# adityamwagh/SuperSLAM

Hardware: AMD Instinct MI355X
Metric: stereo pairs/sec (SPx2+LG) at 1376x376 (higher is better)
Workload: dtype f16; 1 GPU; configs[1]: SuperPoint x2 + select + gather + 1x LightGlue on 1376x376 stereo pairs; a step = 8 x 64 = 512 pairs per GPU resident in HBM (8 library calls of 64 pairs, different images per call), max_keypoints 600, seeded synthetic weights; pairs_per_call=64, max_keypoints=600, matches_last_call=1412, parallelism=replicated weights, pairs sharded over 1 rank(s), no data-path collective

## Files before the change

superslam_amd/csrc/api.hip:

```cpp
#include <algorithm>
#include <atomic>
#include <cmath>
#include <cstdarg>
#include <cstdlib>
#include <cstring>
#include <fstream>
#include <map>
#include <memory>
#include <mutex>
#include <string>
#include <vector>

#include "../../include/sship.h"
#include "../../include/superslam_hip/place_recognizer.hpp"
#include "kernels.h"

namespace sship {

static thread_local std::string g_err;
static void (*g_log_cb)(int, const char*) = nullptr;
static int g_profiling = 0;

void set_error(const std::string& msg) {
  g_err = msg;
// ... 572 lines not shown
}

static int conv_mode() {
  static const int v = [] {
    const char* e = dev_env("SUPERSLAM_HIP_CONV");
    return (SSHIP_DEV_SWITCHES && e && std::string(e) == "strip") ? 2 : 1;
  }();
  return v;
}
static hipError_t conv3(const ConvW& w, const _Float16* in, _Float16* out, int B, int H, int W, bool pool, hipStream_t s) {
#if SSHIP_DEV_SWITCHES
  static const bool wino = [] { const char* e = dev_env("SUPERSLAM_HIP_CONV64"); return e && std::string(e) == "wino"; }();
  if (wino && w.w_wino && sp_conv3x3_wino_fits(H, W, w.cin, w.cout)) return sp_conv3x3_wino(w.w_wino, w.bias, in, out, B, H, W, pool, s);
  return conv_mode() == 1 ? sp_conv3x3_pp(w, in, out, B, H, W, pool, s) : sp_conv3x3_strip(w, in, out, B, H, W, pool, s);
#else
  return sp_conv3x3_pp(w, in, out, B, H, W, pool, s);
#endif
}
static bool conv2_fused(int B, int H2, int W2) {
#if SSHIP_DEV_SWITCHES
  static const std::string mode = [] { const char* e = dev_env("SUPERSLAM_HIP_CONV2"); return std::string(e ? e : ""); }();
  static const bool other = [] { const char* e = dev_env("SUPERSLAM_HIP_CONV64"); return e != nullptr; }();
  if (mode == "split" || other || conv_mode() != 1) return false;
#endif
  return sp_conv2ab_fused_fits(B, H2, W2, true);
}
static hipError_t conv3a_layer(const ConvW& w, const _Float16* in, _Float16* out, int B, int H, int W, hipStream_t s) {
#if SSHIP_DEV_SWITCHES
  static const bool roll = [] { const char* e = dev_env("SUPERSLAM_HIP_CONV3A"); return e && std::string(e) == "roll"; }();
  if (roll && conv_mode() == 1 && w.cin == 64 && w.cout == 128 && w.ct == 64 && sp_conv3a_roll_fits(B, H, W)) return sp_conv3a_roll(w, in, out, B, H, W, s);
#endif
  return conv3(w, in, out, B, H, W, false, s);
}
static hipError_t conv1ab(sship_sp* sp, const uint8_t* img, _Float16* out, int B, int H, int W, hipStream_t s);
static bool desc_dense_mode() {
  static const bool v = [] { const char* e = dev_env("SUPERSLAM_HIP_DESC"); return e && std::string(e) == "dense"; }();
  return v;
}
static hipError_t desc_head(sship_sp* sp, int img0, int Hc, int Wc, const int* cell_h, const int* cell_w, const int* n_dev, int B,
                            _Float16* out, size_t out_img_stride, hipStream_t s) {
  const int mk = sp->cfg.max_keypoints;
  if (desc_dense_mode()) {
    launch_desc_head_gather(sp->cDb32, sp->aDa.as<_Float16>() + (size_t)img0 * Hc * Wc * 256, Hc, Wc, cell_h, cell_w, n_dev, mk, B, out,
                            out_img_stride, s);
    return hipGetLastError();
  }
  return launch_desc_head_sparse(sp->cDa, sp->cDb32, sp->a4b.as<_Float16>() + (size_t)img0 * Hc * Wc * 128, Hc, Wc, cell_h, cell_w, n_dev,
                                 mk, B, out, out_img_stride, s);
}

static int sp_network(sship_sp* sp, const uint8_t* imgs, int B, int H, int W, hipStream_t s, bool dense_desc) {
  int H2, W2, H4, W4, Hc, Wc;
  sp_shapes(H, W, H2, W2, H4, W4, Hc, Wc);
  SSHIP_HIP_CHECK(conv1ab(sp, imgs, sp->a1b.as<_Float16>(), B, H, W, s));
  g_timer.mark_fine("sp_gpu_infer:encoder/conv1a+conv1b+pool", s);
  if (conv2_fused(B, H2, W2)) {
    SSHIP_HIP_CHECK(sp_conv2ab_fused(sp->c2a, sp->c2b, sp->a1b.as<_Float16>(), sp->a2b.as<_Float16>(), B, H2, W2, s));
    g_timer.mark_fine("sp_gpu_infer:encoder/conv2a+conv2b+pool", s);
  } else {
    SSHIP_HIP_CHECK(conv3(sp->c2a, sp->a1b.as<_Float16>(), sp->a2a.as<_Float16>(), B, H2, W2, false, s));
    g_timer.mark_fine("sp_gpu_infer:encoder/conv2a", s);
    SSHIP_HIP_CHECK(conv3(sp->c2b, sp->a2a.as<_Float16>(), sp->a2b.as<_Float16>(), B, H2, W2, true, s));
    g_timer.mark_fine("sp_gpu_infer:encoder/conv2b+pool", s);
  }
  SSHIP_HIP_CHECK(conv3a_layer(sp->c3a, sp->a2b.as<_Float16>(), sp->a3a.as<_Float16>(), B, H4, W4, s));
  g_timer.mark_fine("sp_gpu_infer:encoder/conv3a", s);
  SSHIP_HIP_CHECK(conv3(sp->c3b, sp->a3a.as<_Float16>(), sp->a3b.as<_Float16>(), B, H4, W4, true, s));
  g_timer.mark_fine("sp_gpu_infer:encoder/conv3b+pool", s);
  SSHIP_HIP_CHECK(conv3(sp->c4a, sp->a3b.as<_Float16>(), sp->a4a.as<_Float16>(), B, Hc, Wc, false, s));
  g_timer.mark_fine("sp_gpu_infer:encoder/conv4a", s);
  SSHIP_HIP_CHECK(conv3(sp->c4b, sp->a4a.as<_Float16>(), sp->a4b.as<_Float16>(), B, Hc, Wc, false, s));
  g_timer.mark(g_profiling >= 2 ? "sp_gpu_infer:encoder/conv4b" : "sp_gpu_infer:encoder", s);
  SSHIP_HIP_CHECK(conv3(sp->cPa, sp->a4b.as<_Float16>(), sp->aPa.as<_Float16>(), B, Hc, Wc, false, s));
  g_timer.mark_fine("sp_gpu_infer:heads/convPa", s);
  SSHIP_HIP_CHECK(sp_conv1x1_f32(sp->cPb, sp->aPa.as<_Float16>(), sp->logits.as<float>(), kLogitStride, B, Hc, Wc, s));
  if (dense_desc || desc_dense_mode()) SSHIP_HIP_CHECK(conv3(sp->cDa, sp->a4b.as<_Float16>(), sp->aDa.as<_Float16>(), B, Hc, Wc, false, s));
  if (dense_desc) SSHIP_HIP_CHECK(sp_conv1x1_f16(sp->cDb, sp->aDa.as<_Float16>(), sp->draw.as<_Float16>(), B, Hc, Wc, s));
  g_timer.mark(g_profiling >= 2 ? "sp_gpu_infer:heads/convPb" : "sp_gpu_infer:heads", s);
  return SSHIP_OK;
}

static int sp_select(sship_sp* sp, int B, int H, int W, float* scores_out, float* kp_out, int* n_out, hipStream_t s) {
  int H2, W2, H4, W4, Hc, Wc;
  sp_shapes(H, W, H2, W2, H4, W4, Hc, Wc);
  if (sp->cand_zero_ptr != sp->cand_count.p || sp->cand_zero_n < B || sp->cand_zero_stream != s)
    SSHIP_HIP_CHECK(hipMemsetAsync(sp->cand_count.p, 0, (size_t)B * 4, s));
  sp->cand_zero_ptr = sp->cand_count.p; sp->cand_zero_n = 0; sp->cand_zero_stream = s;
  NmsArgs a{};
  a.logits = sp->logits.as<float>(); a.ls = kLogitStride; a.B = B; a.H = Hc * 8; a.W = Wc * 8;
  a.radius = sp->cfg.nms_radius; a.thr_f = sp->thr_f; a.border = sp->cfg.remove_borders;
  a.cand = sp->cand.as<unsigned long long>(); a.cand_count = sp->cand_count.as<int>(); a.cap = sp->cap;
  a.scores_out = scores_out;
  launch_nms_tile(0, a, s);
  g_timer.mark_fine("sp_extract_stereo:select/nms_tile", s);
  TopkArgs t{};
  t.cand = a.cand; t.cand_count = a.cand_count; t.cap = sp->cap; t.max_kp = sp->cfg.max_keypoints;
  t.score_w = Wc * 8;
  t.scale_x = static_cast<float>(W) / (Wc * 8);
  t.scale_y = static_cast<float>(H) / (Hc * 8);
  t.desc_h = Hc; t.desc_w = Wc; t.kp_xys = kp_out; t.cell_h = sp->cell_h.as<int>(); t.cell_w = sp->cell_w.as<int>();
  t.n_out = n_out; t.n_cand_out = nullptr; t.reset_count = a.cand_count;
  launch_topk(t, B, s);
  SSHIP_HIP_CHECK(hipGetLastError());
  sp->cand_zero_n = B;
  g_timer.mark(g_profiling >= 2 ? "sp_extract_stereo:select/topk" : "sp_extract_stereo:select", s);
  return SSHIP_OK;
}

static hipError_t conv1ab(sship_sp* sp, const uint8_t* img, _Float16* out, int B, int H, int W, hipStream_t s) {
#if SSHIP_DEV_SWITCHES
  if (conv_mode() == 2) return sp_conv1ab_fused(sp->c1b, sp->w1a_frag, sp->b1a, img, out, B, H, W, s);
// ... 73 lines not shown
          const _Float16 hi = (_Float16)b->data[co];
          f[4] = hi;
          f[5] = (_Float16)(b->data[co] - (float)hi);
        }
      }
    SSHIP_HIP_CHECK(hipMalloc(reinterpret_cast<void**>(&sp->w1a_fragb), fr.size() * sizeof(_Float16)));
    SSHIP_HIP_CHECK(hipMemcpy(sp->w1a_fragb, fr.data(), fr.size() * sizeof(_Float16), hipMemcpyHostToDevice));
  }
  SSHIP_HIP_CHECK(hipStreamCreateWithFlags(&sp->stream, hipStreamDefault));
  if (int rc = sship_pool_create(sp->cfg.pool_slots, sp->cfg.max_keypoints, SSHIP_DESC_DIM, &sp->pool)) return rc;
  *out = sp.release();
  return SSHIP_OK;
}
extern "C" void sship_sp_destroy(sship_sp* sp) {
  bind_thread();
  if (!sp) return;
  (void)hipDeviceSynchronize();
  for (ConvW* c : {&sp->c1b, &sp->c2a, &sp->c2b, &sp->c3a, &sp->c3b, &sp->c4a, &sp->c4b, &sp->cPa, &sp->cPb, &sp->cDa, &sp->cDb, &sp->cDb32})
    free_conv(*c);
  if (sp->w1a) (void)hipFree(sp->w1a);
  if (sp->b1a) (void)hipFree(sp->b1a);
  if (sp->w1a_frag) (void)hipFree(sp->w1a_frag);
  if (sp->w1a_fragb) (void)hipFree(sp->w1a_fragb);
  ring_free(sp);
  if (sp->pool) sship_pool_destroy(sp->pool);
  sp->pool = nullptr;
  if (sp->stream) (void)hipStreamDestroy(sp->stream);
  delete sp;
}
extern "C" int sship_sp_debug_activation(sship_sp* sp, int layer, void* out_host, unsigned long long bytes) {
  bind_thread();
  if (!sp || !out_host) return fail(SSHIP_ERR_INVALID, "sp_debug_activation: null argument");
  DevBuf* bufs[8] = {nullptr, &sp->a1b, &sp->a2a, &sp->a2b, &sp->a3a, &sp->a3b, &sp->a4a, &sp->a4b};
  if (layer < 1 || layer > 7 || !bufs[layer]->p || bytes > bufs[layer]->bytes) return fail(SSHIP_ERR_INVALID, "sp_debug_activation: bad layer / size");
  SSHIP_HIP_CHECK(hipDeviceSynchronize());
  SSHIP_HIP_CHECK(hipMemcpy(out_host, bufs[layer]->p, bytes, hipMemcpyDeviceToHost));
  return SSHIP_OK;
}
extern "C" sship_pool* sship_sp_pool(sship_sp* sp) {
  bind_thread(); return sp ? sp->pool : nullptr; }
extern "C" int sship_sp_max_keypoints(const sship_sp* sp) { return sp ? sp->cfg.max_keypoints : 0; }

extern "C" int sship_sp_extract_batch_device(sship_sp* sp, const uint8_t* imgs, int batch, int h, int w, void* desc_out,
                                             float* kp_out, int* n_out, void* stream) {
  bind_thread();
  if (!sp || !imgs || !desc_out || !kp_out || !n_out || batch <= 0) return fail(SSHIP_ERR_INVALID, "sp_extract_batch_device: bad arguments");
  hipStream_t s = static_cast<hipStream_t>(stream);
  if (int rc = sp_ensure(sp, batch, h, w)) return rc;
  if (g_profiling && imgs != sp->img.as<uint8_t>())
    SSHIP_HIP_CHECK(hipMemcpyAsync(sp->img.p, imgs, (size_t)batch * h * w, hipMemcpyDeviceToDevice, s));
  sp->img_valid = g_profiling != 0 || imgs == sp->img.as<uint8_t>();
  g_timer.begin(s);
  if (int rc = sp_network(sp, imgs, batch, h, w, s, false)) return rc;
  if (int rc = sp_select(sp, batch, h, w, nullptr, kp_out, n_out, s)) return rc;
  int H2, W2, H4, W4, Hc, Wc;
  sp_shapes(h, w, H2, W2, H4, W4, Hc, Wc);
  SSHIP_HIP_CHECK(desc_head(sp, 0, Hc, Wc, sp->cell_h.as<int>(), sp->cell_w.as<int>(), n_out, batch, static_cast<_Float16*>(desc_out),
                            (size_t)sp->cfg.max_keypoints * 256, s));
  g_timer.mark("sp_extract_stereo:gather", s);
  return SSHIP_OK;
}

extern "C" int sship_sp_dense(sship_sp* sp, const uint8_t* imgs, int batch, int h, int w, float* scores, void* desc_grid,
                              float* logits, void* stream) {
  bind_thread();
  if (!sp || !imgs || batch <= 0) return fail(SSHIP_ERR_INVALID, "sp_dense: bad arguments");
  hipStream_t s = static_cast<hipStream_t>(stream);
  if (int rc = sp_ensure(sp, batch, h, w)) return rc;
  if (int rc = sp_network(sp, imgs, batch, h, w, s, desc_grid != nullptr)) return rc;
  int H2, W2, H4, W4, Hc, Wc;
  sp_shapes(h, w, H2, W2, H4, W4, Hc, Wc);
  if (scores) {
    NmsArgs a{};
    a.logits = sp->logits.as<float>(); a.ls = kLogitStride; a.B = batch; a.H = Hc * 8; a.W = Wc * 8;
    a.radius = sp->cfg.nms_radius; a.scores_out = scores;
    launch_nms_tile(0, a, s);
  }
  if (desc_grid) launch_desc_dense_chw(sp->draw.as<_Float16>(), Hc * Wc, batch, static_cast<_Float16*>(desc_grid), s);
  if (logits) launch_logits_chw(sp->logits.as<float>(), kLogitStride, Hc * Wc, batch, logits, s);
  SSHIP_HIP_CHECK(hipGetLastError());
  return SSHIP_OK;
}

extern "C" int sship_mfma_probe(int random_operands, float* tflops) {
  bind_thread();
  if (!tflops) return fail(SSHIP_ERR_INVALID, "mfma_probe: null argument");
  if (int rc = require_device()) return rc;
  SSHIP_HIP_CHECK(mfma_probe(random_operands != 0, tflops));
  return SSHIP_OK;
}

extern "C" int sship_sp_bench_layer(sship_sp* sp, int layer, int batch, int h, int w, int iters, float* avg_ms,
                                    double* macs) {
  bind_thread();
  if (!sp || !avg_ms || iters <= 0 || layer < 0 || layer > 15) return fail(SSHIP_ERR_INVALID, "sp_bench_layer: bad arguments");
  if (batch > sp->wsB || h != sp->wsH || w != sp->wsW) return fail(SSHIP_ERR_INVALID, "sp_bench_layer: run the network at this shape first");
  if (layer <= 1 && !sp->img_valid)
    return fail(SSHIP_ERR_INVALID, "sp_bench_layer: the handle holds no copy of the last input - make one call with sship_set_profiling(1) first "
                                   "(a launch on stale / zero pixels runs at a higher clock than the real one)");
  int H2, W2, H4, W4, Hc, Wc;
  sp_shapes(h, w, H2, W2, H4, W4, Hc, Wc);
  hipStream_t s = sp->stream;
  _Float16 *a1a = sp->a1a.as<_Float16>(), *a1b = sp->a1b.as<_Float16>(), *a2a = sp->a2a.as<_Float16>(),
           *a2b = sp->a2b.as<_Float16>(), *a3a = sp->a3a.as<_Float16>(), *a3b = sp->a3b.as<_Float16>(),
           *a4a = sp->a4a.as<_Float16>(), *a4b = sp->a4b.as<_Float16>(), *aPa = sp->aPa.as<_Float16>(),
           *aDa = sp->aDa.as<_Float16>();
  auto run = [&]() -> hipError_t {
    switch (layer) {
      case 0: launch_conv1a(sp->img.as<uint8_t>(), sp->w1a, sp->b1a, a1a, batch, h, w, s); return hipGetLastError();
      case 1: return conv1ab(sp, sp->img.as<uint8_t>(), a1b, batch, h, w, s);
      case 15:
        if (!sp_conv2ab_fused_fits(batch, H2, W2, true)) return hipErrorInvalidValue;
        return sp_conv2ab_fused(sp->c2a, sp->c2b, a1b, a2b, batch, H2, W2, s);
      case 2: return conv3(sp->c2a, a1b, a2a, batch, H2, W2, false, s);
      case 3: return conv3(sp->c2b, a2a, a2b, batch, H2, W2, true, s);
      case 4: return conv3a_layer(sp->c3a, a2b, a3a, batch, H4, W4, s);
      case 5: return conv3(sp->c3b, a3a, a3b, batch, H4, W4, true, s);
      case 6: return conv3(sp->c4a, a3b, a4a, batch, Hc, Wc, false, s);
      case 7: return conv3(sp->c4b, a4a, a4b, batch, Hc, Wc, false, s);
      case 8: return conv3(sp->cPa, a4b, aPa, batch, Hc, Wc, false, s);
      case 9: return sp_conv1x1_f32(sp->cPb, aPa, sp->logits.as<float>(), kLogitStride, batch, Hc, Wc, s);
      case 10: return conv3(sp->cDa, a4b, aDa, batch, Hc, Wc, false, s);
      case 11: return sp_conv1x1_f16(sp->cDb, aDa, sp->draw.as<_Float16>(), batch, Hc, Wc, s);
      case 12: {
        if (hipError_t e = hipMemsetAsync(sp->cand_count.p, 0, (size_t)batch * 4, s)) return e;
        sp->cand_zero_n = 0;
        NmsArgs a{};
        a.logits = sp->logits.as<float>(); a.ls = kLogitStride; a.B = batch; a.H = Hc * 8; a.W = Wc * 8;
        a.radius = sp->cfg.nms_radius; a.thr_f = sp->thr_f; a.border = sp->cfg.remove_borders;
        a.cand = sp->cand.as<unsigned long long>(); a.cand_count = sp->cand_count.as<int>(); a.cap = sp->cap;
        launch_nms_tile(0, a, s);
        return hipGetLastError();
      }
      case 13: {
        TopkArgs t{};
        t.cand = sp->cand.as<unsigned long long>(); t.cand_count = sp->cand_count.as<int>(); t.cap = sp->cap;
        t.max_kp = sp->cfg.max_keypoints; t.score_w = Wc * 8;
        t.scale_x = static_cast<float>(w) / (Wc * 8); t.scale_y = static_cast<float>(h) / (Hc * 8);
        t.desc_h = Hc; t.desc_w = Wc; t.kp_xys = sp->kp.as<float>(); t.cell_h = sp->cell_h.as<int>(); t.cell_w = sp->cell_w.as<int>();
        t.n_out = sp->n_dev.as<int>(); t.n_cand_out = nullptr;
        launch_topk(t, batch, s);
        return hipGetLastError();
      }
      default:
        if (hipError_t e = sp->desc_stage.ensure((size_t)batch * sp->cfg.max_keypoints * 512)) return e;
        return desc_head(sp, 0, Hc, Wc, sp->cell_h.as<int>(), sp->cell_w.as<int>(), sp->n_dev.as<int>(), batch, sp->desc_stage.as<_Float16>(),
                         (size_t)sp->cfg.max_keypoints * 256, s);
    }
  };
  if (layer == 13 || layer == 14) {
    const int keep = layer;
    layer = 12; SSHIP_HIP_CHECK(run());
    layer = 13; SSHIP_HIP_CHECK(run());
    layer = keep;
  }
  const double px[12] = {(double)h * w, (double)h * w, (double)H2 * W2, (double)H2 * W2, (double)H4 * W4, (double)H4 * W4,
                         (double)Hc * Wc, (double)Hc * Wc, (double)Hc * Wc, (double)Hc * Wc, (double)Hc * Wc, (double)Hc * Wc};
  const double mpp[12] = {9.0 * 64, 576.0 * 64 + 9.0 * 64 , 576.0 * 64, 576.0 * 64, 576.0 * 128, 1152.0 * 128, 1152.0 * 128,
                          1152.0 * 128, 1152.0 * 256, 256.0 * 65, 1152.0 * 256, 256.0 * 256};
  if (macs) *macs = layer < 12 ? px[layer] * mpp[layer] * batch : layer == 15 ? (px[2] * mpp[2] + px[3] * mpp[3]) * batch : 0.0;
  SSHIP_HIP_CHECK(run());
  hipEvent_t e0, e1;
  SSHIP_HIP_CHECK(hipEventCreate(&e0));
  SSHIP_HIP_CHECK(hipEventCreate(&e1));
  SSHIP_HIP_CHECK(hipEventRecord(e0, s));
  for (int i = 0; i < iters; ++i) SSHIP_HIP_CHECK(run());
  SSHIP_HIP_CHECK(hipEventRecord(e1, s));
  SSHIP_HIP_CHECK(hipEventSynchronize(e1));
  float ms = 0.f;
  SSHIP_HIP_CHECK(hipEventElapsedTime(&ms, e0, e1));
  (void)hipEventDestroy(e0); (void)hipEventDestroy(e1);
  *avg_ms = ms / iters;
  return SSHIP_OK;
}

static int sp_extract_device(sship_sp* sp, const uint8_t* gray, int B, int h, int w, sship_features* const* outs);
static int sp_extract_host(sship_sp* sp, const uint8_t* const* imgs, int B, int h, int w, int stride, int channels,
                           sship_features* const* outs) {
  if (channels != 1 && channels != 3) return fail(SSHIP_ERR_INVALID, "image must have 1 or 3 channels");
  if (h <= 0 || w <= 0 || stride < w * channels) return fail(SSHIP_ERR_INVALID, "bad image geometry");
  if (int rc = sp_ensure(sp, B, h, w)) return rc;
  hipStream_t s = sp->stream;
  const size_t row = (size_t)w * channels, img_bytes = row * h;
  uint8_t* hp = sp->h_img.as<uint8_t>();
  for (int b = 0; b < B; ++b)
    for (int y = 0; y < h; ++y) memcpy(hp + b * img_bytes + y * row, imgs[b] + (size_t)y * stride, row);
  if (channels == 1) {
    SSHIP_HIP_CHECK(hipMemcpyAsync(sp->img.p, hp, img_bytes * B, hipMemcpyHostToDevice, s));
  } else {
    SSHIP_HIP_CHECK(hipMemcpyAsync(sp->gray_in.p, hp, img_bytes * B, hipMemcpyHostToDevice, s));
    launch_bgr2gray(sp->gray_in.as<uint8_t>(), B * h * w, sp->img.as<uint8_t>(), s);
  }
  sp->img_valid = true;
// ... 952 lines not shown
```

superslam_amd/csrc/conv_pp128.hip:

```cpp
#include "igemm.h"
#include "kernels.h"

#include <cstdio>
#include <cstdlib>
#include <string>
#include <type_traits>
#include <vector>

#ifndef SSHIP_PP_PRIO
#define SSHIP_PP_PRIO 2
#endif
#ifndef SSHIP_PP_TRACE_BUILD
#define SSHIP_PP_TRACE_BUILD 0
#endif

#ifndef SSHIP_PP128_ABL
#define SSHIP_PP128_ABL 0
#endif
#ifndef SSHIP_PP128_COLMAJOR
#define SSHIP_PP128_COLMAJOR 0
#endif

namespace sship {

// ... 773 lines not shown
    if (!tbuf) (void)hipMalloc(&tbuf, 4096 * 2 * 6 * 8);
    (void)hipMemsetAsync(tbuf, 0, 4096 * 2 * 6 * 8, s);
    b.trace = tbuf;
  }
  hipLaunchKernelGGL(kern, dim3(gx, ncb), dim3(512), smem, s, b);
  if (trace_on) {
    std::vector<unsigned long long> h(4096 * 2 * 6);
    (void)hipStreamSynchronize(s);
    (void)hipMemcpy(h.data(), tbuf, h.size() * 8, hipMemcpyDeviceToHost);
    double sum[6] = {0}; long cnt = 0;
    for (int i = 0; i < gx * ncb * 2; ++i) {
      if (!h[i * 6 + 3]) continue;
      for (int k = 0; k < 6; ++k) sum[k] += (double)h[i * 6 + k];
      ++cnt;
    }
    if (cnt) fprintf(stderr, "[pp128w trace cin=%d cout=%d pool=%d] dma issue=%.0f dma wait=%.0f | mfma=%.0f | barrier wait after data=%.0f after mfma=%.0f (clk, %ld groups)\n",
                     NCH * 32, a.cout, (int)POOL, sum[0] / cnt, sum[1] / cnt, sum[3] / cnt, sum[4] / cnt, sum[5] / cnt, cnt);
  }
  return hipGetLastError();
}

bool sp_conv3x3_pp128_fits(int B, int H, int W, int cin) { return (size_t)B * H * W * cin * 2 + (size_t)(W + 1) * cin * 4 + 8192 < 0x7f000000ull; }

hipError_t sp_conv3x3_pp128(const ConvW& w, const _Float16* in, _Float16* out, int B, int H, int W, bool pool, hipStream_t s) {
  if ((w.cin != 128 && w.cin != 64) || !w.w_q || w.cout % 64 || !sp_conv3x3_pp128_fits(B, H, W, w.cin)) return hipErrorInvalidValue;
  Pp128Args a{};
  a.in = in; a.wpack = w.w_q; a.bias = w.bias; a.out = out; a.B = B; a.H = H; a.W = W; a.cout = w.cout;
  if (w.cin == 64) return pool ? launch_pp128w<true, 2>(a, s) : launch_pp128w<false, 2>(a, s);
  static const bool th8 = [] { const char* e = dev_env("SUPERSLAM_HIP_CONV128"); return e && std::string(e) == "th8"; }();
  if (th8) return pool ? launch_pp128<true>(a, s) : launch_pp128<false>(a, s);
  return pool ? launch_pp128w<true, 4>(a, s) : launch_pp128w<false, 4>(a, s);
}

}
```

superslam_amd/csrc/kernels.h:

```cpp
#pragma once
#include "common.h"

namespace sship {

constexpr int kMaxKp = 4096;
constexpr int kLogitStride = 68;

void launch_conv1a(const uint8_t* img, const float* w, const float* bias, _Float16* out, int B, int H, int W,
                   hipStream_t s);
struct NmsArgs {
  const float* logits;
  int ls;
  const float* scores_in;
  int B, H, W;
  int radius;
  float thr_f;
  int border;
  unsigned long long* cand;
  int* cand_count;
  int cap;
  float* scores_out;
  float* scores_raw_out;
};
float threshold_as_float(double thr);
// ... 9 lines not shown
  int desc_h, desc_w;
  float* kp_xys;
  int* cell_h;
  int* cell_w;
  int* n_out;
  int* n_cand_out;
};
void launch_topk(const TopkArgs& a, int B, hipStream_t s);
void launch_threshold_scan(const float* scores, int H, int W, float thr_f, int border, unsigned long long* cand,
                           int* cand_count, int cap, hipStream_t s);
void launch_gather_hwc(bool raw, const _Float16* grid, int C, int gh, int gw, size_t img_stride, const int* cell_h,
                       const int* cell_w, const int* n_dev, int n_host, int max_kp, int B, _Float16* out,
                       hipStream_t s);
void launch_gather_chw(const _Float16* grid, int C, int gh, int gw, const int* cell_h, const int* cell_w, int n,
                       _Float16* out, hipStream_t s);
void launch_desc_dense_chw(const _Float16* raw, int cells_per_img, int B, _Float16* out, hipStream_t s);
void launch_logits_chw(const float* in, int ls, int cells_per_img, int B, float* out, hipStream_t s);
void launch_bgr2gray(const uint8_t* in, int n, uint8_t* out, hipStream_t s);

struct ConvW {
  _Float16* w = nullptr;
  _Float16* w_wino = nullptr;
  _Float16* w_q = nullptr;
  float* bias = nullptr;
  int cin = 0, cout = 0, cout_pad = 0, ks = 1, ct = 64;
};
hipError_t sp_conv3x3_strip(const ConvW& w, const _Float16* in, _Float16* out, int B, int H, int W, bool pool,
                            hipStream_t s);
hipError_t sp_conv1ab_fused(const ConvW& w1b, const _Float16* w1a_frag, const float* b1a, const uint8_t* img,
                            _Float16* out, int B, int H, int W, hipStream_t s);
hipError_t sp_conv3x3_pp(const ConvW& w, const _Float16* in, _Float16* out, int B, int H, int W, bool pool, hipStream_t s);
bool sp_conv3x3_pp128_fits(int B, int H, int W, int cin);
hipError_t sp_conv3x3_pp128(const ConvW& w, const _Float16* in, _Float16* out, int B, int H, int W, bool pool, hipStream_t s);
bool sp_conv2ab_fused_fits(int B, int H, int W, bool any_batch);
hipError_t sp_conv2ab_fused(const ConvW& wa, const ConvW& wb, const _Float16* in, _Float16* out, int B, int H, int W, hipStream_t s);
bool sp_conv3a_roll_fits(int B, int H, int W);
hipError_t sp_conv3a_roll(const ConvW& w, const _Float16* in, _Float16* out, int B, int H, int W, hipStream_t s);
hipError_t sp_conv1ab_pp(const ConvW& w1b, const _Float16* w1a_frag, const float* b1a, const uint8_t* img, _Float16* out,
                         int B, int H, int W, hipStream_t s);
bool sp_conv3x3_wino_fits(int H, int W, int cin, int cout);
hipError_t sp_conv3x3_wino(const _Float16* upack, const float* bias, const _Float16* in, _Float16* out, int B, int H, int W, bool pool, hipStream_t s);
hipError_t sp_conv1x1_f16(const ConvW& w, const _Float16* in, _Float16* out, int B, int H, int W, hipStream_t s);
int cu_count();

hipError_t mfma_probe(bool random_operands, float* tflops);

hipError_t launch_desc_head_sparse(const ConvW& da32, const ConvW& db32, const _Float16* a4b, int Hc, int Wc, const int* cell_h,
                                   const int* cell_w, const int* n_dev, int max_kp, int B, _Float16* out, size_t out_img_stride,
                                   hipStream_t s);
void launch_desc_head_gather(const ConvW& db32, const _Float16* da, int Hc, int Wc, const int* cell_h, const int* cell_w,
                             const int* n_dev, int max_kp, int B, _Float16* out, size_t out_img_stride, hipStream_t s);
hipError_t sp_conv1x1_f32(const ConvW& w, const _Float16* in, float* out, int ostride, int B, int H, int W,
                          hipStream_t s);

hipError_t ep_conv(const ConvW& w, const _Float16* in, _Float16* out, const _Float16* res, int H, int W, bool relu, bool decim,
                   hipStream_t s, float* ws = nullptr, size_t ws_bytes = 0);
size_t ep_splitk_workspace_bytes(int in_h, int in_w);
void launch_ep_resize_norm(const uint8_t* src, int stride, int ch, const int* tab, int out_w, int out_h, float* out, hipStream_t s);
void launch_ep_im2col(const float* x, int H, int W, int Ho, int Wo, _Float16* out, hipStream_t s);
void launch_ep_maxpool(const _Float16* in, int H, int W, int Ho, int Wo, _Float16* out, hipStream_t s);
void launch_ep_stem_pool(const float* x, int H, int W, int Ho, int Wo, int Hp, int Wp, const _Float16* wfrag, const float* bias, _Float16* out,
                         hipStream_t s);
size_t ep_tail_ws_floats();
void launch_ep_tail(const _Float16* feat, int npix, float p, const float* wt, const float* bias, float* ws, int* counters, float* out,
                    hipStream_t s);

// ... 26 lines not shown
```

Before: 5618 pairs/s.

## Fuse SuperPoint detector head convPa and convPb into one kernel

Adds a fused kernel that runs the 3x3 convPa (128->256, ReLU) and feeds its tile results straight from registers into the 1x1 convPb (256->65) via MFMA, writing fp32 logits directly. This removes the write and re-read of the 256-channel aPa intermediate in HBM and one kernel launch. The fused kernel uses a large LDS footprint, warp-specialised DMA/MFMA roles and a smaller row tile, so occupancy and per-tile efficiency may differ from the tuned standalone conv. It is enabled by default when shapes fit, with env switches to fall back.

```diff
diff --git a/superslam_amd/csrc/api.hip b/superslam_amd/csrc/api.hip
--- a/superslam_amd/csrc/api.hip
+++ b/superslam_amd/csrc/api.hip
@@ -628,6 +628,14 @@
 #endif
   return conv3(w, in, out, B, H, W, false, s);
 }
+static bool convp_fused(const sship_sp* sp, int B, int Hc, int Wc) {
+#if SSHIP_DEV_SWITCHES
+  static const std::string mode = [] { const char* e = dev_env("SUPERSLAM_HIP_CONVP"); return std::string(e ? e : ""); }();
+  static const bool other = [] { return dev_env("SUPERSLAM_HIP_CONV128") != nullptr || dev_env("SUPERSLAM_HIP_CONVPB") != nullptr; }();
+  if (mode == "split" || (mode != "fused" && (other || conv_mode() != 1))) return false;
+#endif
+  return sp_convpab_fits(sp->cPa, sp->cPb, B, Hc, Wc, kLogitStride);
+}
 static hipError_t conv1ab(sship_sp* sp, const uint8_t* img, _Float16* out, int B, int H, int W, hipStream_t s);
 static bool desc_dense_mode() {
   static const bool v = [] { const char* e = dev_env("SUPERSLAM_HIP_DESC"); return e && std::string(e) == "dense"; }();
@@ -667,12 +675,17 @@
   g_timer.mark_fine("sp_gpu_infer:encoder/conv4a", s);
   SSHIP_HIP_CHECK(conv3(sp->c4b, sp->a4a.as<_Float16>(), sp->a4b.as<_Float16>(), B, Hc, Wc, false, s));
   g_timer.mark(g_profiling >= 2 ? "sp_gpu_infer:encoder/conv4b" : "sp_gpu_infer:encoder", s);
-  SSHIP_HIP_CHECK(conv3(sp->cPa, sp->a4b.as<_Float16>(), sp->aPa.as<_Float16>(), B, Hc, Wc, false, s));
-  g_timer.mark_fine("sp_gpu_infer:heads/convPa", s);
-  SSHIP_HIP_CHECK(sp_conv1x1_f32(sp->cPb, sp->aPa.as<_Float16>(), sp->logits.as<float>(), kLogitStride, B, Hc, Wc, s));
+  const bool fused_p = convp_fused(sp, B, Hc, Wc);
+  if (fused_p) {
+    SSHIP_HIP_CHECK(sp_convpab(sp->cPa, sp->cPb, sp->a4b.as<_Float16>(), sp->logits.as<float>(), kLogitStride, B, Hc, Wc, s));
+  } else {
+    SSHIP_HIP_CHECK(conv3(sp->cPa, sp->a4b.as<_Float16>(), sp->aPa.as<_Float16>(), B, Hc, Wc, false, s));
+    g_timer.mark_fine("sp_gpu_infer:heads/convPa", s);
+    SSHIP_HIP_CHECK(sp_conv1x1_f32(sp->cPb, sp->aPa.as<_Float16>(), sp->logits.as<float>(), kLogitStride, B, Hc, Wc, s));
+  }
   if (dense_desc || desc_dense_mode()) SSHIP_HIP_CHECK(conv3(sp->cDa, sp->a4b.as<_Float16>(), sp->aDa.as<_Float16>(), B, Hc, Wc, false, s));
   if (dense_desc) SSHIP_HIP_CHECK(sp_conv1x1_f16(sp->cDb, sp->aDa.as<_Float16>(), sp->draw.as<_Float16>(), B, Hc, Wc, s));
-  g_timer.mark(g_profiling >= 2 ? "sp_gpu_infer:heads/convPb" : "sp_gpu_infer:heads", s);
+  g_timer.mark(g_profiling < 2 ? "sp_gpu_infer:heads" : fused_p ? "sp_gpu_infer:heads/convPa+convPb" : "sp_gpu_infer:heads/convPb", s);
   return SSHIP_OK;
 }
 
@@ -812,9 +825,10 @@
   bind_thread();
   if (!sp || !out_host) return fail(SSHIP_ERR_INVALID, "sp_debug_activation: null argument");
   DevBuf* bufs[8] = {nullptr, &sp->a1b, &sp->a2a, &sp->a2b, &sp->a3a, &sp->a3b, &sp->a4a, &sp->a4b};
-  if (layer < 1 || layer > 7 || !bufs[layer]->p || bytes > bufs[layer]->bytes) return fail(SSHIP_ERR_INVALID, "sp_debug_activation: bad layer / size");
+  DevBuf* buf = layer >= 1 && layer <= 7 ? bufs[layer] : layer == 16 ? &sp->logits : nullptr;
+  if (!buf || !buf->p || bytes > buf->bytes) return fail(SSHIP_ERR_INVALID, "sp_debug_activation: bad layer / size");
   SSHIP_HIP_CHECK(hipDeviceSynchronize());
-  SSHIP_HIP_CHECK(hipMemcpy(out_host, bufs[layer]->p, bytes, hipMemcpyDeviceToHost));
+  SSHIP_HIP_CHECK(hipMemcpy(out_host, buf->p, bytes, hipMemcpyDeviceToHost));
   return SSHIP_OK;
 }
 extern "C" sship_pool* sship_sp_pool(sship_sp* sp) {
@@ -873,7 +887,7 @@
 extern "C" int sship_sp_bench_layer(sship_sp* sp, int layer, int batch, int h, int w, int iters, float* avg_ms,
                                     double* macs) {
   bind_thread();
-  if (!sp || !avg_ms || iters <= 0 || layer < 0 || layer > 15) return fail(SSHIP_ERR_INVALID, "sp_bench_layer: bad arguments");
+  if (!sp || !avg_ms || iters <= 0 || layer < 0 || layer > 16) return fail(SSHIP_ERR_INVALID, "sp_bench_layer: bad arguments");
   if (batch > sp->wsB || h != sp->wsH || w != sp->wsW) return fail(SSHIP_ERR_INVALID, "sp_bench_layer: run the network at this shape first");
   if (layer <= 1 && !sp->img_valid)
     return fail(SSHIP_ERR_INVALID, "sp_bench_layer: the handle holds no copy of the last input - make one call with sship_set_profiling(1) first "
@@ -900,6 +914,8 @@
       case 7: return conv3(sp->c4b, a4a, a4b, batch, Hc, Wc, false, s);
       case 8: return conv3(sp->cPa, a4b, aPa, batch, Hc, Wc, false, s);
       case 9: return sp_conv1x1_f32(sp->cPb, aPa, sp->logits.as<float>(), kLogitStride, batch, Hc, Wc, s);
+      case 16:
+        return sp_convpab(sp->cPa, sp->cPb, a4b, sp->logits.as<float>(), kLogitStride, batch, Hc, Wc, s);
       case 10: return conv3(sp->cDa, a4b, aDa, batch, Hc, Wc, false, s);
       case 11: return sp_conv1x1_f16(sp->cDb, aDa, sp->draw.as<_Float16>(), batch, Hc, Wc, s);
       case 12: {
@@ -938,7 +954,8 @@
                          (double)Hc * Wc, (double)Hc * Wc, (double)Hc * Wc, (double)Hc * Wc, (double)Hc * Wc, (double)Hc * Wc};
   const double mpp[12] = {9.0 * 64, 576.0 * 64 + 9.0 * 64 , 576.0 * 64, 576.0 * 64, 576.0 * 128, 1152.0 * 128, 1152.0 * 128,
                           1152.0 * 128, 1152.0 * 256, 256.0 * 65, 1152.0 * 256, 256.0 * 256};
-  if (macs) *macs = layer < 12 ? px[layer] * mpp[layer] * batch : layer == 15 ? (px[2] * mpp[2] + px[3] * mpp[3]) * batch : 0.0;
+  if (macs) *macs = layer < 12 ? px[layer] * mpp[layer] * batch : layer == 15 ? (px[2] * mpp[2] + px[3] * mpp[3]) * batch
+                   : layer == 16 ? (px[8] * mpp[8] + px[9] * mpp[9]) * batch : 0.0;
   SSHIP_HIP_CHECK(run());
   hipEvent_t e0, e1;
   SSHIP_HIP_CHECK(hipEventCreate(&e0));
diff --git a/superslam_amd/csrc/conv_pp128.hip b/superslam_amd/csrc/conv_pp128.hip
--- a/superslam_amd/csrc/conv_pp128.hip
+++ b/superslam_amd/csrc/conv_pp128.hip
@@ -829,4 +829,388 @@
   return pool ? launch_pp128w<true, 4>(a, s) : launch_pp128w<false, 4>(a, s);
 }
 
+
+constexpr int S_TH = 8, S_THH = 10;
+constexpr int S_IN_UNITS = S_THH * Q_TWH * 4;
+constexpr int S_IN_DMA = (S_IN_UNITS + 63) / 64;
+constexpr int S_IN_HALFS = S_IN_DMA * 64 * 8;
+constexpr int S_DMA_PER_WAVE = 6;
+constexpr int S_PB_HALFS = 8 * 5 * 512;
+constexpr int S_NPASS = 4;
+constexpr size_t S_SMEM = (size_t)(2 * Q_W_SLOT + 2 * S_IN_HALFS + S_PB_HALFS) * 2 + (2 * 256 + 80) * 4;
+static_assert(S_SMEM <= 163840, "LDS budget");
+
+struct PabArgs {
+  const _Float16* in;
+  const _Float16* wpack;
+  const float* bias;
+  const _Float16* wb;
+  const float* bias_b;
+  float* out;
+  int B, H, W, ostride;
+};
+
+__global__ __launch_bounds__(512, 2) void conv3x3_pab(PabArgs p) {
+  constexpr int MT = 2, NT = 2, PB = 256;
+  extern __shared__ __attribute__((aligned(16))) char smem_pab[];
+  _Float16* s_w = reinterpret_cast<_Float16*>(smem_pab);
+  const int tid = threadIdx.x, wave = tid >> 6, lane = tid & 63, j = lane & 31, hh = lane >> 5, kb = lane >> 4;
+  const int grp = __builtin_amdgcn_readfirstlane(wave >> 2);
+  const int gw = wave & 3;
+  const int gw_u = __builtin_amdgcn_readfirstlane(gw);
+  _Float16* my_in = s_w + 2 * Q_W_SLOT + grp * S_IN_HALFS;
+  _Float16* s_pb = s_w + 2 * Q_W_SLOT + 2 * S_IN_HALFS;
+  float* s_bias = reinterpret_cast<float*>(s_pb + S_PB_HALFS);
+  float* s_bias_b = s_bias + 2 * 256;
+
+  const int tiles_x = (p.W + Q_TW - 1) / Q_TW, tiles_y = (p.H + S_TH - 1) / S_TH;
+  const bool pairs = pp128w_pairs_shape(false, p.B, p.W);
+  const int txn = tiles_x - 1, we = p.W - txn * Q_TW;
+  const int tiles_xv = pairs ? 2 * txn + 1 : tiles_x, nb_walk = pairs ? p.B / 2 : p.B;
+  const int ntiles = nb_walk * tiles_xv * tiles_y;
+  const int t_begin = (int)((long long)blockIdx.x * ntiles / gridDim.x);
+  const int t_end = (int)((long long)(blockIdx.x + 1) * ntiles / gridDim.x);
+  const int n_wg = t_end - t_begin;
+  if (n_wg <= 0) return;
+  const _Float16* wsrc = p.wpack;
+
+  for (int u = tid; u < Q_W_SLOT / 8; u += 512) *reinterpret_cast<uint4*>(s_w + u * 8) = *reinterpret_cast<const uint4*>(wsrc + u * 8);
+  for (int u = tid; u < S_PB_HALFS / 8; u += 512) {
+    const int ks = u / 320, mt = (u >> 6) % 5, l = u & 63;
+    *reinterpret_cast<uint4*>(s_pb + u * 8) = *reinterpret_cast<const uint4*>(p.wb + (size_t)(16 * mt + (l & 15)) * 256 + ks * 32 + (l >> 4) * 8);
+  }
+  s_bias[tid] = p.bias[tid & 255];
+  if (tid < 80) s_bias_b[tid] = tid < 65 ? p.bias_b[tid] : 0.f;
+  const unsigned lane16 = lane * 16;
+  const int dma_f0 = gw_u < 2 ? gw_u * 5 : 10 + (gw_u - 2) * 4;
+  auto fill_weights = [&](int wi, int half) __attribute__((always_inline)) {
+    const unsigned long long ga = (unsigned long long)(uintptr_t)(wsrc + (size_t)wi * Q_W_SLOT + (half * 18 + dma_f0) * 512);
+    const unsigned long long g = (unsigned long long)(unsigned)__builtin_amdgcn_readfirstlane((unsigned)ga) |
+                                 ((unsigned long long)(unsigned)__builtin_amdgcn_readfirstlane((unsigned)(ga >> 32)) << 32);
+    const unsigned dst = __builtin_amdgcn_readfirstlane((unsigned)(uintptr_t)(s_w + (wi & 1) * Q_W_SLOT + (half * 18 + dma_f0) * 512));
+    unsigned keep;
+    asm volatile("s_mov_b32 %0, m0\n\ts_mov_b32 m0, %2\n\ts_nop 0\n\t"
+                 "global_load_lds_dwordx4 %1, %3\n\t"
+                 "global_load_lds_dwordx4 %1, %3 offset:1024\n\t"
+                 "global_load_lds_dwordx4 %1, %3 offset:2048\n\t"
+                 "global_load_lds_dwordx4 %1, %3 offset:3072\n\t"
+                 "s_mov_b32 m0, %0"
+                 : "=&s"(keep) : "v"(lane16), "s"(dst), "s"(g) : "memory");
+    if (gw_u < 2)
+      asm volatile("s_mov_b32 %0, m0\n\ts_mov_b32 m0, %2\n\ts_nop 0\n\tglobal_load_lds_dwordx4 %1, %3\n\ts_mov_b32 m0, %0"
+                   : "=&s"(keep) : "v"(lane16), "s"(dst + 4096), "s"(g + 4096) : "memory");
+  };
+  int boff[3][2];
+#pragma unroll
+  for (int kx = 0; kx < 3; ++kx)
+#pragma unroll
+    for (int ksl = 0; ksl < 2; ++ksl) boff[kx][ksl] = (j + kx) * 32 + (((2 * ksl + hh) ^ (((j + kx) >> 2) & 3)) << 3);
+
+  auto walk_init = [&](int t) __attribute__((always_inline)) {
+    TileWalk w;
+    w.tx = t % tiles_xv;
+    const int r = t / tiles_xv;
+    w.ty = r % tiles_y; w.b = r / tiles_y;
+    return w;
+  };
+  auto walk_next = [&](TileWalk& w) __attribute__((always_inline)) {
+    w.tx += 2;
+    while (w.tx >= tiles_xv) {
+      w.tx -= tiles_xv;
+      if (++w.ty == tiles_y) { w.ty = 0; ++w.b; }
+    }
+  };
+  auto decode = [&](const TileWalk& w, int& img, int& tx, bool& shared) __attribute__((always_inline)) {
+    if (!pairs) { img = w.b; tx = w.tx; shared = false; return; }
+    shared = w.tx == 2 * txn;
+    const int second = !shared && w.tx >= txn;
+    img = 2 * w.b + second;
+    tx = shared ? txn : w.tx - second * txn;
+  };
+  TileWalk pw = walk_init(t_begin + grp), ew = pw;
+
+  unsigned voff[S_DMA_PER_WAVE];
+  unsigned m_top = 0, m_bot = 0, m_left = 0, m_right = 0;
+  unsigned m_second = 0, m_dead = 0;
+  {
+    const int px = (gw * S_DMA_PER_WAVE) * 16 + (lane >> 2);
+    int r = (px * 241) >> 13;
+    int c = px - r * Q_TWH;
+    const int rhi_last = min(S_THH - 1, p.H - (tiles_y - 1) * S_TH), chi_last = min(Q_TWH - 1, p.W - (tiles_x - 1) * Q_TW);
+#pragma unroll
+    for (int i = 0; i < S_DMA_PER_WAVE; ++i) {
+      const int u = (lane & 3) ^ ((c >> 2) & 3);
+      voff[i] = r < S_THH ? (unsigned)(4096 - (i & 3) * 1024 + (r * p.W + c) * PB + u * 16) : R_OOB;
+      m_top |= (r >= 1 ? 1u : 0u) << i;
+      m_bot |= (r <= rhi_last ? 1u : 0u) << i;
+      m_left |= (c >= 1 ? 1u : 0u) << i;
+      m_right |= (c <= chi_last ? 1u : 0u) << i;
+      m_second |= (c >= we + 2 && c < 2 * we + 3 ? 1u : 0u) << i;
+      m_dead |= (c == we + 1 || c >= 2 * we + 3 ? 1u : 0u) << i;
+      c += 16;
+      if (c >= Q_TWH) { c -= Q_TWH; ++r; }
+    }
+  }
+  rsrc4_t rs;
+  {
+    const unsigned long long ba = (unsigned long long)(uintptr_t)p.in - (unsigned long long)(p.W + 1) * (unsigned long long)PB - 4096ull;
+    rs[0] = __builtin_amdgcn_readfirstlane((int)(unsigned)ba);
+    rs[1] = __builtin_amdgcn_readfirstlane((int)((unsigned)(ba >> 32) & 0xffffu));
+    rs[2] = 0x7ffffff0;
+    rs[3] = 0x00020000;
+  }
+  const unsigned lds_in0 = __builtin_amdgcn_readfirstlane((unsigned)(uintptr_t)(my_in + (gw_u * S_DMA_PER_WAVE) * 512));
+  auto dma_in = [&](int chunk, bool last) __attribute__((always_inline)) {
+    int img, txr;
+    bool shared;
+    decode(pw, img, txr, shared);
+    const int y0 = pw.ty * S_TH, x0 = txr * Q_TW;
+    const unsigned soff = __builtin_amdgcn_readfirstlane((unsigned)((img * p.H + y0) * p.W + x0) * (unsigned)PB + (unsigned)chunk * 64u);
+    const bool interior = !shared && y0 >= 1 && y0 + S_TH + 1 <= p.H && x0 >= 1 && x0 + Q_TW + 1 <= p.W;
+    unsigned v[S_DMA_PER_WAVE];
+    if (shared) {
+      unsigned ok = 0x3fu & ~m_dead;
+      if (pw.ty == 0) ok &= m_top;
+      if (pw.ty == tiles_y - 1) ok &= m_bot;
+      const unsigned delta = (unsigned)(p.H * p.W - (we + 2)) * (unsigned)PB;
+#pragma unroll
+      for (int i = 0; i < S_DMA_PER_WAVE; ++i) v[i] = (ok >> i) & 1u ? voff[i] + ((m_second >> i) & 1u ? delta : 0u) : R_OOB;
+    } else {
+      unsigned ok = 0x3fu;
+      if (!interior) {
+        if (pw.ty == 0) ok &= m_top;
+        if (pw.ty == tiles_y - 1) ok &= m_bot;
+        if (txr == 0) ok &= m_left;
+        if (txr == tiles_x - 1) ok &= m_right;
+      }
+#pragma unroll
+      for (int i = 0; i < S_DMA_PER_WAVE; ++i) v[i] = (ok >> i) & 1u ? voff[i] : R_OOB;
+    }
+    unsigned keep;
+    asm volatile("s_mov_b32 %0, m0\n\ts_mov_b32 m0, %5\n\ts_nop 0\n\t"
+                 "buffer_load_dwordx4 %1, %6, %7 offen lds\n\t"
+                 "buffer_load_dwordx4 %2, %6, %7 offen offset:1024 lds\n\t"
+                 "buffer_load_dwordx4 %3, %6, %7 offen offset:2048 lds\n\t"
+                 "buffer_load_dwordx4 %4, %6, %7 offen offset:3072 lds\n\t"
+                 "s_mov_b32 m0, %0"
+                 : "=&s"(keep) : "v"(v[0]), "v"(v[1]), "v"(v[2]), "v"(v[3]), "s"(lds_in0), "s"(rs), "s"(soff) : "memory");
+    if (gw_u < 3)
+      asm volatile("s_mov_b32 %0, m0\n\ts_mov_b32 m0, %3\n\ts_nop 0\n\t"
+                   "buffer_load_dwordx4 %1, %4, %5 offen lds\n\t"
+                   "buffer_load_dwordx4 %2, %4, %5 offen offset:1024 lds\n\t"
+                   "s_mov_b32 m0, %0"
+                   : "=&s"(keep) : "v"(v[4]), "v"(v[5]), "s"(lds_in0 + 4096u), "s"(rs), "s"(soff) : "memory");
+    if (last) walk_next(pw);
+  };
+
+  f16x_t acc[MT][NT];
+  f4x_t lg[NT][2][5];
+  auto mfma_item = [&](auto chunk_c, int pass) __attribute__((always_inline)) {
+    constexpr int chunk = decltype(chunk_c)::value;
+    const _Float16* wc = s_w + (chunk & 1) * Q_W_SLOT + lane * 8;
+    const _Float16* ib = my_in + (gw * 2) * Q_TWH * 32;
+    h8_t af[3][MT], rows[8];
+    auto load_a = [&](int s_, int buf) __attribute__((always_inline)) {
+      const int t = s_ / 3, ky = s_ - 3 * t, kx = t >> 1, ksl = t & 1, idx = (ky * 3 + kx) * 2 + ksl;
+#pragma unroll
+      for (int m = 0; m < MT; ++m) af[buf][m] = *reinterpret_cast<const h8_t*>(wc + (idx * MT + m) * 512);
+    };
+    auto load_row = [&](int t, int row) __attribute__((always_inline)) {
+      rows[(4 * t + row) & 7] = *reinterpret_cast<const h8_t*>(ib + row * Q_TWH * 32 + boff[t >> 1][t & 1]);
+    };
+#pragma unroll
+    for (int row = 0; row < 4; ++row) load_row(0, row);
+    load_a(0, 0);
+    load_a(1, 1);
+    if constexpr (chunk == 0) {
+#pragma unroll
+      for (int m = 0; m < MT; ++m)
+#pragma unroll
+        for (int n = 0; n < NT; ++n)
+#pragma unroll
+          for (int g = 0; g < 4; ++g) {
+            const float4 b4 = *reinterpret_cast<const float4*>(s_bias + n * 256 + pass * 64 + m * 32 + hh * 4 + g * 8);
+            acc[m][n][4 * g + 0] = b4.x; acc[m][n][4 * g + 1] = b4.y; acc[m][n][4 * g + 2] = b4.z; acc[m][n][4 * g + 3] = b4.w;
+          }
+    }
+#pragma unroll
+    for (int s_ = 0; s_ < 18; ++s_) {
+      const int t = s_ / 3, ky = s_ - 3 * t;
+      if (s_ + 2 < 18) load_a(s_ + 2, (s_ + 2) % 3);
+      if (t + 1 < 6) {
+        if (ky == 0) { load_row(t + 1, 0); load_row(t + 1, 1); }
+        else load_row(t + 1, ky + 1);
+      }
+      __builtin_amdgcn_sched_barrier(0);
+#pragma unroll
+      for (int n = 0; n < NT; ++n)
+#pragma unroll
+        for (int m = 0; m < MT; ++m) acc[m][n] = mfma32(af[s_ % 3][m], rows[(4 * t + n + ky) & 7], acc[m][n]);
+      __builtin_amdgcn_sched_barrier(0);
+    }
+  };
+  auto pass_end = [&](int pass) __attribute__((always_inline)) {
+    const h2_t z2 = {(_Float16)0.f, (_Float16)0.f};
+    auto relu2 = [&](float lo, float hi) __attribute__((always_inline)) -> unsigned {
+      h2_t v = {(_Float16)lo, (_Float16)hi};
+      v = __builtin_elementwise_max(v, z2);
+      return *reinterpret_cast<const unsigned*>(&v);
+    };
+    if (pass == 0) {
+#pragma unroll
+      for (int n = 0; n < NT; ++n)
+#pragma unroll
+        for (int h = 0; h < 2; ++h)
+#pragma unroll
+          for (int mt = 0; mt < 5; ++mt) lg[n][h][mt] = *reinterpret_cast<const f4x_t*>(s_bias_b + 16 * mt + 4 * kb);
+    }
+#pragma unroll
+    for (int m = 0; m < MT; ++m) {
+      h8_t pa[5];
+#pragma unroll
+      for (int mt = 0; mt < 5; ++mt) pa[mt] = *reinterpret_cast<const h8_t*>(s_pb + (((2 * pass + m) * 5 + mt) * 64 + lane) * 8);
+#pragma unroll
+      for (int n = 0; n < NT; ++n) {
+        const f16x_t& a = acc[m][n];
+        unsigned q[4][2];
+#pragma unroll
+        for (int g = 0; g < 4; ++g)
+#pragma unroll
+          for (int d = 0; d < 2; ++d) q[g][d] = relu2(a[4 * g + 2 * d], a[4 * g + 2 * d + 1]);
+        unsigned x[4], y[4];
+#pragma unroll
+        for (int d = 0; d < 2; ++d) {
+          const auto rx = __builtin_amdgcn_permlane32_swap(q[0][d], q[2][d], false, false);
+          const auto ry = __builtin_amdgcn_permlane32_swap(q[1][d], q[3][d], false, false);
+          x[d] = rx[0]; x[2 + d] = rx[1];
+          y[d] = ry[0]; y[2 + d] = ry[1];
+        }
+        typedef unsigned u4_t __attribute__((ext_vector_type(4)));
+        u4_t b0, b1;
+#pragma unroll
+        for (int d = 0; d < 4; ++d) {
+          const auto r = __builtin_amdgcn_permlane16_swap(x[d], y[d], false, false);
+          b0[d] = r[0]; b1[d] = r[1];
+        }
+        const h8_t f0 = __builtin_bit_cast(h8_t, b0), f1 = __builtin_bit_cast(h8_t, b1);
+#pragma unroll
+        for (int mt = 0; mt < 5; ++mt) {
+          lg[n][0][mt] = __builtin_amdgcn_mfma_f32_16x16x32_f16(pa[mt], f0, lg[n][0][mt], 0, 0, 0);
+          lg[n][1][mt] = __builtin_amdgcn_mfma_f32_16x16x32_f16(pa[mt], f1, lg[n][1][mt], 0, 0, 0);
+        }
+      }
+    }
+    if (pass == S_NPASS - 1) {
+      int b0, txr;
+      bool shared;
+      decode(ew, b0, txr, shared);
+      const int y0 = ew.ty * S_TH, x0 = txr * Q_TW;
+      walk_next(ew);
+#pragma unroll
+      for (int n = 0; n < NT; ++n) {
+        const int y = y0 + gw * 2 + n;
+#pragma unroll
+        for (int h = 0; h < 2; ++h) {
+          const int jj = 16 * h + (lane & 15);
+          const bool second = shared && jj >= we + 2;
+          const int b = b0 + second;
+          const int x = second ? x0 + jj - (we + 2) : (shared && jj >= we ? p.W : x0 + jj);
+          if (y < p.H && x < p.W) {
+            float* o = p.out + ((size_t)(b * p.H + y) * p.W + x) * p.ostride + 4 * kb;
+#pragma unroll
+            for (int mt = 0; mt < 4; ++mt) *reinterpret_cast<f4x_t*>(o + 16 * mt) = lg[n][h][mt];
+            if (kb == 0) o[64] = lg[n][h][4][0];
+          }
+        }
+      }
+    }
+  };
+
+  const int T0 = (n_wg + 1) >> 1, T1 = n_wg >> 1;
+  auto data_role = [&](int wi, int dma_half, int in_chunk, bool last) __attribute__((always_inline)) {
+    if (SSHIP_PP_PRIO) __builtin_amdgcn_s_setprio(SSHIP_PP_PRIO);
+    if (in_chunk >= 0) dma_in(in_chunk, last);
+    if (wi >= 0) fill_weights(wi, dma_half);
+    if (SSHIP_PP_PRIO) __builtin_amdgcn_s_setprio(0);
+    asm volatile("s_waitcnt vmcnt(0)" ::: "memory");
+    __syncthreads();
+  };
+  auto mfma_role = [&](auto chunk_c, int pass) __attribute__((always_inline)) {
+    constexpr int chunk = decltype(chunk_c)::value;
+    mfma_item(chunk_c, pass);
+    if constexpr (chunk == Q_NCHUNK - 1) pass_end(pass);
+    __syncthreads();
+  };
+  const std::integral_constant<int, 0> c0{};
+  const std::integral_constant<int, 1> c1{};
+  const std::integral_constant<int, 2> c2{};
+  const std::integral_constant<int, 3> c3{};
+  __syncthreads();
+  if (grp == 0) {
+    data_role(-1, 0, T0 > 0 ? 0 : -1, false);
+#pragma unroll 1
+    for (int it = 0; it < T0; ++it) {
+      const bool more = it + 1 < T0;
+#pragma unroll 1
+      for (int pass = 0; pass < S_NPASS; ++pass) {
+        const int w0 = pass * 4;
+        const bool lastp = pass == S_NPASS - 1;
+        mfma_role(c0, pass);
+        data_role(w0 + 1, 1, 1, false);
+        mfma_role(c1, pass);
+        data_role(w0 + 2, 1, 2, false);
+        mfma_role(c2, pass);
+        data_role(w0 + 3, 1, 3, lastp);
+        mfma_role(c3, pass);
+        data_role((w0 + 4) & 15, 1, (!lastp || more) ? 0 : -1, false);
+      }
+    }
+  } else {
+    __syncthreads();
+#pragma unroll 1
+    for (int it = 0; it < T1; ++it) {
+#pragma unroll 1
+      for (int pass = 0; pass < S_NPASS; ++pass) {
+        const int w0 = pass * 4;
+        data_role(w0 + 1, 0, 0, false);
+        mfma_role(c0, pass);
+        data_role(w0 + 2, 0, 1, false);
+        mfma_role(c1, pass);
+        data_role(w0 + 3, 0, 2, false);
+        mfma_role(c2, pass);
+        data_role((w0 + 4) & 15, 0, 3, pass == S_NPASS - 1);
+        mfma_role(c3, pass);
+      }
+    }
+    if (T0 > T1) {
+#pragma unroll 1
+      for (int k = 0; k < S_NPASS * Q_NCHUNK; ++k) {
+        data_role((k + 1) & 15, 0, -1, false);
+        __syncthreads();
+      }
+    }
+  }
 }
+
+bool sp_convpab_fits(const ConvW& pa, const ConvW& pb, int B, int H, int W, int ostride) {
+  return pa.cin == 128 && pa.cout == 256 && pa.w_q && pb.cin == 256 && pb.cout == 65 && pb.w_q && ostride >= 68 && ostride % 4 == 0 &&
+         B >= 1 && H >= 1 && W >= 1 && sp_conv3x3_pp128_fits(B, H, W, 128);
+}
+
+hipError_t sp_convpab(const ConvW& pa, const ConvW& pb, const _Float16* in, float* logits, int ostride, int B, int H, int W, hipStream_t s) {
+  if (!sp_convpab_fits(pa, pb, B, H, W, ostride)) return hipErrorInvalidValue;
+  static const hipError_t attr_rc = hipFuncSetAttribute(reinterpret_cast<const void*>(conv3x3_pab), hipFuncAttributeMaxDynamicSharedMemorySize, (int)S_SMEM);
+  if (attr_rc != hipSuccess) return attr_rc;
+  PabArgs a{};
+  a.in = in; a.wpack = pa.w_q; a.bias = pa.bias; a.wb = pb.w_q; a.bias_b = pb.bias; a.out = logits;
+  a.B = B; a.H = H; a.W = W; a.ostride = ostride;
+  const int tiles_x = (W + Q_TW - 1) / Q_TW;
+  const int ntiles = (pp128w_pairs_shape(false, B, W) ? B / 2 * (2 * (tiles_x - 1) + 1) : B * tiles_x) * ((H + S_TH - 1) / S_TH);
+  int gx = cu_count();
+  if (gx * 2 > ntiles) gx = (ntiles + 1) / 2;
+  if (gx < 1) gx = 1;
+  hipLaunchKernelGGL(conv3x3_pab, dim3(gx), dim3(512), S_SMEM, s, a);
+  return hipGetLastError();
+}
+
+}
diff --git a/superslam_amd/csrc/kernels.h b/superslam_amd/csrc/kernels.h
--- a/superslam_amd/csrc/kernels.h
+++ b/superslam_amd/csrc/kernels.h
@@ -65,6 +65,8 @@
 hipError_t sp_conv3x3_pp(const ConvW& w, const _Float16* in, _Float16* out, int B, int H, int W, bool pool, hipStream_t s);
 bool sp_conv3x3_pp128_fits(int B, int H, int W, int cin);
 hipError_t sp_conv3x3_pp128(const ConvW& w, const _Float16* in, _Float16* out, int B, int H, int W, bool pool, hipStream_t s);
+bool sp_convpab_fits(const ConvW& pa, const ConvW& pb, int B, int H, int W, int ostride);
+hipError_t sp_convpab(const ConvW& pa, const ConvW& pb, const _Float16* in, float* logits, int ostride, int B, int H, int W, hipStream_t s);
 bool sp_conv2ab_fused_fits(int B, int H, int W, bool any_batch);
 hipError_t sp_conv2ab_fused(const ConvW& wa, const ConvW& wb, const _Float16* in, _Float16* out, int B, int H, int W, hipStream_t s);
 bool sp_conv3a_roll_fits(int B, int H, int W);
```

Result: faster. 5690 pairs/s (median of 6 runs) (+1.3%).
